# luisrui/Multimodal-Relation-Extrapolation

Hardware: AMD Instinct MI355X
Metric: scored triples/sec + hit@10 parity, FB15K-237-ZS TransE d=200 at 1/2/4/8 MI355X (higher is better)
Workload: dtype f32; 1 GPU; C2 FB15K-237-ZS TransE d=200 p=1 norm_flag, filtered link prediction; n_entities=14208, dim=200, n_sweeps=35192

## Files before the change

multimodal-relation-extrapolation_amd/csrc/link.hip:

```cpp
#include <stdlib.h>

#include <algorithm>
#include <map>
#include <mutex>
#include <tuple>
#include <type_traits>

#include "mmre_common.h"

namespace mmre {

typedef float f32x2 __attribute__((ext_vector_type(2)));

constexpr int TQ = 128;
constexpr int TE = 128;
constexpr int KC = 8;
constexpr int NT = 256;

constexpr int KS_MFMA = 16;
__host__ __device__ inline int n_planes(int model) { return (model == MMRE_COMPLEX || model == MMRE_ROTATE) ? 2 : 1; }
__host__ __device__ inline bool mfma_model(int model) { return model == MMRE_DISTMULT || model == MMRE_COMPLEX; }
inline int plane_rows(int model, int dim) {
  return (int)round_up(dim, !mfma_model(model) ? KC : KS_MFMA / n_planes(model));
}
// ... 655 lines not shown
                                                     const int64_t* __restrict__ off, const int32_t* __restrict__ ids,
                                                     const float* __restrict__ list_v,
                                                     const int32_t* __restrict__ qtrue, const float* __restrict__ thr,
                                                     const int64_t* __restrict__ qr, const int8_t* __restrict__ qmode,
                                                     int64_t n_query, int64_t n_ent,
                                                     const uint32_t* __restrict__ type_head,
                                                     const uint32_t* __restrict__ type_tail, int64_t type_words,
                                                     int32_t* __restrict__ counts) {
  __shared__ __attribute__((aligned(16))) int32_t s_id[64];
  __shared__ __attribute__((aligned(16))) float s_v[64];
  __shared__ __attribute__((aligned(16))) int32_t s_tb[64];
  const int tid = threadIdx.x;
  for (int64_t g = blockIdx.x; g < n_groups; g += gridDim.x) {
    const int64_t qa = grp_qoff[g], qb = grp_qoff[g + 1];
    const int64_t la = off[g], lb = off[g + 1];
    const int64_t q0 = grp_q[qa];
    const uint32_t* tm = type_head ? (qmode[q0] == MMRE_HEAD_BATCH ? type_head : type_tail) : nullptr;
    const int64_t r = qr[q0];
    for (int64_t qc = qa; qc < qb; qc += 64) {
      const int64_t qi = qc + tid;
      const bool active = qi < qb;
      const int64_t q = active ? grp_q[qi] : 0;
      const int32_t tr = active ? qtrue[q] : -1;
      const float th = active ? thr[q] : 0.0f;
      int c = 0, cc = 0;
      for (int64_t lc = la; lc < lb; lc += 64) {
        const int nl = (int)((lb - lc) < 64 ? (lb - lc) : 64);
        __syncthreads();
        {
          int32_t id = -1, tb = 0;
          float v = 0.0f;
          if (tid < nl) {
            const int64_t j = ids[lc + tid];
            if (j >= 0 && j < n_ent) {
              id = (int32_t)j;
              v = list_v[lc + tid];
              tb = tm ? (int32_t)type_bit(tm, type_words, r, j) : 0;
            }
          }
          s_id[tid] = id;
          s_v[tid] = v;
          s_tb[tid] = tb;
        }
        __syncthreads();
        if (active) {
          for (int i = 0; i < nl; i += 4) {
            const int4 e = *reinterpret_cast<const int4*>(&s_id[i]);
            const float4 v = *reinterpret_cast<const float4*>(&s_v[i]);
            const int4 t = *reinterpret_cast<const int4*>(&s_tb[i]);
            const int b0 = (e.x >= 0) & (e.x != tr) & (v.x < th);
            const int b1 = (e.y >= 0) & (e.y != tr) & (v.y < th);
            const int b2 = (e.z >= 0) & (e.z != tr) & (v.z < th);
            const int b3 = (e.w >= 0) & (e.w != tr) & (v.w < th);
            c += b0 + b1 + b2 + b3;
            cc += (b0 & t.x) + (b1 & t.y) + (b2 & t.z) + (b3 & t.w);
          }
        }
      }
      if (active) {
        counts[0 * n_query + q] = 0;
        counts[1 * n_query + q] = -c;
        counts[2 * n_query + q] = 0;
        counts[3 * n_query + q] = -cc;
      }
    }
  }
}

struct UnitMap {
  int m, r, ex0, el0, n_main, lo0, count, nq;
  bool emajor;
  __device__ __forceinline__ UnitMap(int grp, int n_groups, int n_qt, int n_et, bool emajor_ = false) {
    nq = n_qt;
    emajor = emajor_;
    m = n_et / n_groups;
    r = n_et - m * n_groups;
    ex0 = grp * m;
    el0 = m * n_groups;
    n_main = n_qt * m;
    const int64_t left = (int64_t)n_qt * r;
    lo0 = (int)(left * grp / n_groups);
    count = n_main + (int)(left * (grp + 1) / n_groups) - lo0;
  }
  __device__ __forceinline__ void at(int i, int& qt, int& et) const {
    if (i < n_main) {
      if (emajor) {
        qt = i % nq;
        et = ex0 + i / nq;
      } else {
        qt = i / m;
        et = ex0 + i % m;
      }
    } else {
      const int j = lo0 + (i - n_main);
      qt = j / r;
      et = el0 + j % r;
    }
  }
};

struct BlockMap {
  int count, qin, ein, QB, EB, e_lo, n_e;
  __device__ __forceinline__ BlockMap(int grp, int n_groups, int member, int P, int n_qt, int n_et, int qb, int eb) {
    e_lo = (int)((int64_t)n_et * grp / n_groups);
    const int e_hi = (int)((int64_t)n_et * (grp + 1) / n_groups);
    const int m_e = e_hi - e_lo;
    QB = qb;
    EB = eb;
    qin = member / EB;
    ein = member - qin * EB;
    count = 0;
    n_e = 0;
    if (qin >= QB || m_e <= 0) return;
    n_e = ein < m_e ? (m_e - ein + EB - 1) / EB : 0;
    const int n_q = qin < n_qt ? (n_qt - qin + QB - 1) / QB : 0;
    count = n_q * n_e;
  }
  __device__ __forceinline__ void at(int i, int& qt, int& et) const {
    const int a = i / n_e, b = i - a * n_e;
    qt = a * QB + qin;
    et = e_lo + b * EB + ein;
  }
};

template <int GS>
struct ValuSmemGrp {
  uint32_t g_ts[GS][TQ];
  uint32_t g_tw[GS][TQ];
  int32_t g_mq[GS][TQ];
  uint32_t g_acc[GS][TQ];
};
template <>
struct ValuSmemGrp<0> {};
constexpr int L1Q_GS = 8;
constexpr double L1Q_GROUP_FRAC = 0.6;

template <int NPL, bool TC, bool LIST, int GS = 0>
struct ValuSmem : ValuSmemGrp<GS> {
  float4 sq[2][NPL][KC][TQ / 4];
  float4 se[2][NPL][KC][TE / 4];
  float s_thr[2][GS ? 1 : TQ];
  int32_t s_true[2][GS ? 1 : TQ];
  int32_t s_rel[2][TC ? TQ : 1];
  int8_t s_mode[2][TC ? TQ : 1];
  std::conditional_t<TC, uint16_t, int32_t> s_cnt[TC ? 2 : 1][GS ? 1 : 8][GS ? 1 : NT];
  uint32_t s_unc[NT / 64];
  uint32_t s_ts[2][GS ? 1 : TQ];
  uint32_t s_tw[2][GS ? 1 : TQ];
  int s_unit;
  uint32_t s_tb[TC ? 2 : 1][TC ? TQ : 1][4];
  int2 s_pairs[LIST ? NT / 64 : 1][LIST ? 128 : 1];
};

template <int OP, bool TC, bool STORE, int PK, int NPL, int DYNC, int GS = 0, bool IDX = false>
__device__ __forceinline__ void sweep_valu_body(
    ValuSmem<NPL, TC, (OP == 5 || OP == 6), GS>& sm, const float* __restrict__ ent_km, int64_t e_pad, int64_t n_ent,
    const float* __restrict__ q_km, int64_t q_pad, int64_t n_query, int kp, int n_et, int e_base, int n_groups,
    int pred_kind, float margin, const float* __restrict__ thr, const int32_t* __restrict__ qtrue,
    const int64_t* __restrict__ qr, const int8_t* __restrict__ qmode, const uint32_t* __restrict__ type_head,
    const uint32_t* __restrict__ type_tail, int64_t type_words, int32_t* __restrict__ counts,
    float* __restrict__ scores, const L1Q& l1) {
  static_assert(NPL == ((OP == 2) ? 2 : 1), "planes");
  constexpr bool L1F = OP == 5 || OP == 6;
  constexpr bool w8 = OP == 6;
  constexpr bool FAST = (OP == 2 || L1F) && !STORE;
  constexpr bool GRP = GS > 0;
  static_assert(!GRP || (L1F && PK == 0 && !TC && !STORE), "the grouped sweep is the plain integer filter's");
  static_assert(!IDX || (OP == 0 && PK == 0 && !TC && !STORE && DYNC == 0 && !GRP),
                "the indexed sweep is the plain f32 one");
  auto& sq = sm.sq;
  auto& se = sm.se;
  auto& s_thr = sm.s_thr;
  auto& s_true = sm.s_true;
  auto& s_rel = sm.s_rel;
  auto& s_mode = sm.s_mode;
  auto& s_cnt = sm.s_cnt;

  const int tid = threadIdx.x;
  const int tq = tid >> 4, te = tid & 15;
  const PredSel<PK> pred(pred_kind, margin);
  const int grp = blockIdx.x % n_groups, gmem = blockIdx.x / n_groups;
  const int per_grp = gridDim.x / n_groups;
  const int n_idx = IDX ? __builtin_amdgcn_readfirstlane((int)*l1.route_n) : 0;
  const int n_qt = IDX   ? (n_idx + TQ - 1) / TQ
                   : GRP ? __builtin_amdgcn_readfirstlane(l1.n_rows[GRP ? 1 : 0]) / TQ
                         : (int)(q_pad / TQ);
  const UnitMap um(grp, n_groups, n_qt, n_et);
  const int nkc = kp / KC;
  constexpr bool dyn = DYNC > 0;
  constexpr int ch_log2 = DYNC >= 4 ? 2 : DYNC >= 2 ? 1 : 0;
  constexpr int ch_mask = (1 << ch_log2) - 1;
  const int u0 = dyn ? gmem << ch_log2 : (int)((int64_t)gmem * um.count / per_grp);
  const int u1 = dyn ? um.count : (int)((int64_t)(gmem + 1) * um.count / per_grp);
  if (u0 >= u1) return;

  float l1d = 0.0f, l1f = 0.0f, l1c = 0.0f;
  if constexpr (L1F) {
    l1d = __uint_as_float(__builtin_amdgcn_readfirstlane(__float_as_uint(l1q_delta(l1.hdr, w8 ? 255.0f : 65535.0f))));
    l1f = (float)(l1.kt + 4) * 0x1p-23f * (1.0f + 0x1p-8f);
    l1c = __builtin_fmaf((float)l1.kt * 1.03f, l1d, 0x1p-120f);
  }

  auto load_meta = [&](int qtile, int slot) {
    const int tid = vgpr_opaque(threadIdx.x);
    if (tid < TQ) {
      int64_t q = (int64_t)qtile * TQ + tid;
      bool v = q < n_query;
      if constexpr (IDX) {
        v = q < (int64_t)n_idx;
        q = v ? l1.route_list[q] : 0;
      }
      const float th = v ? thr[q] : -INFINITY;
      s_thr[slot][tid] = th;
      s_true[slot][tid] = v ? qtrue[q] : -1;
      if constexpr (L1F && PK == 0) {
        uint32_t t_sure, t_span;
        const bool tight = w8 && l1.q_l1c != nullptr;
        const int ktm = sgpr_opaque(l1.kt);
        const float md = __uint_as_float(sgpr_opaque(__float_as_uint(l1d)));
        const float mf = (float)(ktm + 4) * 0x1p-23f * (1.0f + 0x1p-8f);
        const float mc = __builtin_fmaf((float)ktm * 1.03f, md, 0x1p-120f);
        l1_int_thresholds(th, tight ? (v ? l1.q_l1c[q] : 0.0f) + 0x1p-120f : mc, md, mf, tight ? 2u * l1.hdr[3] : 0u,
                          t_sure, t_span);
        if constexpr (w8) {
          if (l1.routed != nullptr && v && l1.routed[q]) t_sure = t_span = 0u;
        }
        sm.s_ts[slot][tid] = t_sure;
        sm.s_tw[slot][tid] = t_span;
      }
      if constexpr (TC) {
        s_rel[slot][tid] = v ? (int32_t)qr[q] : 0;
        s_mode[slot][tid] = v ? qmode[q] : 0;
      }
    }
  };

  auto load_meta_grp = [&](int qtile) -> int {
    int m = 0;
    if constexpr (GRP) {
      const int tid = vgpr_opaque(threadIdx.x);
      m = min(__builtin_amdgcn_readfirstlane(l1.tile_m[qtile]), GS);
      const bool tight = w8 && l1.q_l1c != nullptr;
      const int ktm = sgpr_opaque(l1.kt);
      const float md = __uint_as_float(sgpr_opaque(__float_as_uint(l1d)));
      const float mf = (float)(ktm + 4) * 0x1p-23f * (1.0f + 0x1p-8f);
      const float mc = __builtin_fmaf((float)ktm * 1.03f, md, 0x1p-120f);
      const uint32_t om2 = tight ? 2u * l1.hdr[3] : 0u;
      static_assert(NT == 2 * TQ && GS % 2 == 0, "two slots' rows per pass");
      const int r = tid % TQ, s0 = tid / TQ;
      const int64_t row = (int64_t)qtile * TQ + r;
      const int cnt = l1.row_cnt[row];
      const int64_t off = l1.row_off[row];
      const float rc = tight ? l1.q_l1c[row] : 0.0f;
      int q[GS / 2];
      float th[GS / 2];
#pragma unroll
      for (int u = 0; u < GS / 2; ++u) {
        q[u] = -1;
        if (s0 + 2 * u < cnt) {
          const int qq = l1.grp_q[off + s0 + 2 * u];
          q[u] = (uint32_t)qq < (uint32_t)n_query ? qq : -1;
        }
      }
      if constexpr (w8) {
        if (l1.routed != nullptr) {
#pragma unroll
          for (int u = 0; u < GS / 2; ++u)
            if (q[u] >= 0 && l1.routed[q[u]]) q[u] = -1;
        }
      }
#pragma unroll
      for (int u = 0; u < GS / 2; ++u) th[u] = q[u] >= 0 ? thr[q[u]] : -INFINITY;
#pragma unroll
      for (int u = 0; u < GS / 2; ++u) {
        const int sl = s0 + 2 * u;
        if (sl < m) {
          uint32_t t_sure, t_span;
          l1_int_thresholds(th[u], tight ? (q[u] >= 0 ? rc : 0.0f) + 0x1p-120f : mc, md, mf, om2, t_sure, t_span);
          sm.g_ts[GRP ? sl : 0][r] = t_sure;
          sm.g_tw[GRP ? sl : 0][r] = t_span;
          sm.g_mq[GRP ? sl : 0][r] = q[u];
        }
      }
    }
    return m;
  };

  const int srow = tid >> 5, sc4 = tid & 31;
  float4 rq0, re0, rq1, re1;
  int ld_unit = u0, ld_kc = 0, ld_qt, ld_et;
  um.at(u0, ld_qt, ld_et);
  uint32_t rt0 = 0u, rt1 = 0u;
  bool st_new = false;
  int ld_tpar = 1, st_par = 0, ep_par = 0;
  [[maybe_unused]] int iq0 = 0, iq1 = 0, iq2 = 0, iq3 = 0;
  auto gload = [&]() {
    if constexpr (TC) {
      st_new = ld_kc == 0;
      if (st_new) {
        ld_tpar ^= 1;
        st_par = ld_tpar;
        const int tt = vgpr_opaque(threadIdx.x);
        const int rr = tt >> 1, jw = tt & 1;
        const int64_t q = (int64_t)ld_qt * TQ + rr;
        uint32_t w0 = 0u, w1 = 0u;
        if (q < n_query) {
          const uint32_t* tm = (qmode[q] == MMRE_HEAD_BATCH ? type_head : type_tail) + qr[q] * type_words;
          const int64_t wb = (e_base + (int64_t)ld_et * TE) >> 5;
          if (wb + jw < type_words) w0 = tm[wb + jw];
          if (wb + 2 + jw < type_words) w1 = tm[wb + 2 + jw];
        }
        rt0 = w0;
        rt1 = w1;
      }
    }
    const int k = ld_kc * KC + srow;
    const int64_t q0 = (int64_t)ld_qt * TQ, e0 = (int64_t)ld_et * TE;
    const float* qp = q_km + (int64_t)k * q_pad + q0 + sc4 * 4;
    const float* ep = ent_km + (int64_t)k * e_pad + e0 + sc4 * 4;
    if constexpr (IDX) {
      if (ld_kc == 0) {
        const int p0 = (int)q0 + sc4 * 4;
        iq0 = p0 + 0 < n_idx ? l1.route_list[p0 + 0] : 0;
        iq1 = p0 + 1 < n_idx ? l1.route_list[p0 + 1] : 0;
        iq2 = p0 + 2 < n_idx ? l1.route_list[p0 + 2] : 0;
        iq3 = p0 + 3 < n_idx ? l1.route_list[p0 + 3] : 0;
      }
      const float* qk = q_km + (int64_t)k * q_pad;
      rq0 = make_float4(qk[iq0], qk[iq1], qk[iq2], qk[iq3]);
    } else {
      rq0 = *reinterpret_cast<const float4*>(qp);
    }
    re0 = *reinterpret_cast<const float4*>(ep);
    if constexpr (NPL == 2) {
      rq1 = *reinterpret_cast<const float4*>(qp + (int64_t)kp * q_pad);
      re1 = *reinterpret_cast<const float4*>(ep + (int64_t)kp * e_pad);
    }
    if (++ld_kc == nkc) {
      ld_kc = 0;
      if (dyn) {
        ld_unit = ((ld_unit + 1) & ch_mask) != 0 ? ld_unit + 1 : sm.s_unit;
        if (ld_unit < u1) um.at(ld_unit, ld_qt, ld_et);
      } else if (++ld_unit < u1) {
        um.at(ld_unit, ld_qt, ld_et);
      }
    }
  };
  auto swrite = [&](int buf) {
    if constexpr (TC) {
      if (st_new) {
        const int tt = vgpr_opaque(threadIdx.x);
        *reinterpret_cast<uint2*>(&sm.s_tb[st_par][tt >> 1][(tt & 1) * 2]) = make_uint2(rt0, rt1);
      }
    }
    sq[buf][0][srow][sc4] = rq0;
    se[buf][0][srow][sc4] = re0;
    if constexpr (NPL == 2) {
      sq[buf][NPL - 1][srow][sc4] = rq1;
      se[buf][NPL - 1][srow][sc4] = re1;
    }
  };

  float acc[8][8];
#pragma unroll
  for (int i = 0; i < 8; ++i)
#pragma unroll
    for (int j = 0; j < 8; ++j) acc[i][j] = 0.0f;
  f32x2 accp[4][8];
#pragma unroll
  for (int i = 0; i < 4; ++i)
#pragma unroll
    for (int j = 0; j < 8; ++j) accp[i][j] = f32x2{0.0f, 0.0f};
  if constexpr (GRP) {
    for (int idx = tid; idx < GS * TQ; idx += NT) (&sm.g_acc[0][0])[idx] = 0u;
  } else {
#pragma unroll
    for (int i = 0; i < 8; ++i) {
      s_cnt[0][i][tid] = 0;
      if constexpr (TC) s_cnt[TC ? 1 : 0][i][tid] = 0;
    }
  }
  if (L1F && tid < NT / 64) sm.s_unc[tid] = 0u;
  constexpr bool LIST = L1F;
  int list_n = 0;
  uint32_t n_listed = 0;
  auto rescore = [&](int2 p, bool active) {
    const int64_t q = p.x;
    const int e = p.y;
    bool ok = active;
    if (active && ((uint64_t)q >= (uint64_t)n_query || (uint32_t)e >= (uint32_t)n_ent)) {
      if (l1.guard) atomicAdd(l1.guard, 1u);
      ok = false;
    }
    if constexpr (GRP) {
      if (ok && e + e_base == qtrue[q]) ok = false;
      n_listed += (uint32_t)__builtin_popcountll(__ballot(ok));
    }
    bool beat = false;
    if (ok) {
      if (l1.und_q) atomicAdd(&l1.und_q[q], 1u);
      const float th = thr[q];
      const float sx = l1_exact_rows<GRP ? 3 : 5>(l1.q_rows + q * (int64_t)l1.kt,
                                                  l1.ent_rows + (int64_t)(e + e_base) * l1.kt, l1.kt);
      beat = pred(sx) < th;
      if constexpr (TC) {
        const uint32_t* tm = qmode[q] == MMRE_HEAD_BATCH ? type_head : type_tail;
        if (beat && type_bit(tm, type_words, qr[q], e + e_base)) atomicAdd(&counts[2 * n_query + q], 1);
      }
    }
    const int qi = (int)q;
    uint64_t pend = __ballot(beat);
    while (pend) {
      const int leader = __builtin_ctzll(pend);
      const int ql = __builtin_amdgcn_readlane(qi, leader);
      const bool mine = beat && qi == ql;
      const uint64_t same = __ballot(mine);
      if ((int)(threadIdx.x & 63) == leader) atomicAdd(&counts[ql], (int)__builtin_popcountll(same));
      if (mine) beat = false;
      pend &= ~same;
    }
  };

  int cur_qt, cur_et;
  um.at(u0, cur_qt, cur_et);
  int slot = 0;
  uint32_t lo = 0xFFFFFFFFu;
  const int kk_last = L1F ? ((((l1.kt + (w8 ? 3 : 1)) >> (w8 ? 2 : 1)) + (w8 ? 2 : 1)) & ~1) - (nkc - 1) * KC
                          : KC;
  const uint32_t fb_flag = L1F ? l1.hdr[1] : 0u;
  int cur_m = 0;
  if constexpr (GRP) cur_m = load_meta_grp(cur_qt);
  else load_meta(cur_qt, 0);
  gload();
  swrite(0);
  __syncthreads();
  if (L1F && __builtin_amdgcn_readfirstlane(fb_flag) != (w8 ? L1Q_CODES8 : L1Q_CODES16)) return;
  if (dyn && ch_mask == 0) {
    if (tid == 0) sm.s_unit = per_grp + (int)atomicAdd(&l1.wq[grp * L1Q_WQ_STRIDE], 1u);
    __syncthreads();
  }

  constexpr int KKU = 2;
  int buf = 0;
  for (int unit = u0; unit < u1;) {
    int unit_next = unit + 1;
    for (int kc = 0; kc < nkc; ++kc) {
      const bool more = ld_unit < u1;
      if (more) gload();
      const int kk_n = (L1F && kc == nkc - 1) ? kk_last : KC;
#pragma unroll KKU
      for (int kk = 0; kk < kk_n; ++kk) {
        float4 a0 = sq[buf][0][kk][tq], a1 = sq[buf][0][kk][16 + tq];
        float4 x0 = se[buf][0][kk][te], x1 = se[buf][0][kk][16 + te];
        const float qa[8] = {a0.x, a0.y, a0.z, a0.w, a1.x, a1.y, a1.z, a1.w};
        const float xv[8] = {x0.x, x0.y, x0.z, x0.w, x1.x, x1.y, x1.z, x1.w};
        if constexpr (OP == 2 && FAST) {
          float4 b0 = sq[buf][NPL - 1][kk][tq], b1 = sq[buf][NPL - 1][kk][16 + tq];
          float4 y0 = se[buf][NPL - 1][kk][te], y1 = se[buf][NPL - 1][kk][16 + te];
          const f32x2 qa2[4] = {{a0.x, a0.y}, {a0.z, a0.w}, {a1.x, a1.y}, {a1.z, a1.w}};
          const f32x2 qb2[4] = {{b0.x, b0.y}, {b0.z, b0.w}, {b1.x, b1.y}, {b1.z, b1.w}};
          const f32x2 xv2[4] = {{x0.x, x0.y}, {x0.z, x0.w}, {x1.x, x1.y}, {x1.z, x1.w}};
          const f32x2 yv2[4] = {{y0.x, y0.y}, {y0.z, y0.w}, {y1.x, y1.y}, {y1.z, y1.w}};
#pragma unroll
          for (int ip = 0; ip < 4; ++ip)
#pragma unroll
            for (int jp = 0; jp < 4; ++jp) {
              const f32x2 dr0 = qa2[ip] - xv2[jp], dr1 = qa2[ip] - xv2[jp].yx;
              const f32x2 di0 = qb2[ip] - yv2[jp], di1 = qb2[ip] - yv2[jp].yx;
              const f32x2 p0 = dr0 * dr0, p1 = dr1 * dr1;
              const f32x2 v0 = __builtin_elementwise_fma(di0, di0, p0), v1 = __builtin_elementwise_fma(di1, di1, p1);
              const f32x2 m0 = {__builtin_amdgcn_sqrtf(v0.x), __builtin_amdgcn_sqrtf(v0.y)};
              const f32x2 m1 = {__builtin_amdgcn_sqrtf(v1.x), __builtin_amdgcn_sqrtf(v1.y)};
              accp[ip][2 * jp] = accp[ip][2 * jp] + m0;
              accp[ip][2 * jp + 1] = accp[ip][2 * jp + 1] + m1;
            }
        } else if constexpr (OP == 2) {
          float4 b0 = sq[buf][NPL - 1][kk][tq], b1 = sq[buf][NPL - 1][kk][16 + tq];
          float4 y0 = se[buf][NPL - 1][kk][te], y1 = se[buf][NPL - 1][kk][16 + te];
          const float qb[8] = {b0.x, b0.y, b0.z, b0.w, b1.x, b1.y, b1.z, b1.w};
          const float yv[8] = {y0.x, y0.y, y0.z, y0.w, y1.x, y1.y, y1.z, y1.w};
          float v[8], y[8];
#pragma unroll
          for (int j = 0; j < 8; ++j) {
            const float dr = qa[0] - xv[j], di = qb[0] - yv[j];
            v[j] = __builtin_fmaf(di, di, dr * dr);
// ... 208 lines not shown
            }
            s_cnt[0][i][tid] += c;
            if constexpr (TC) s_cnt[TC ? 1 : 0][i][tid] += cc;
          }
          if constexpr (LIST) {
            int2* wl = sm.s_pairs[tid >> 6];
            const int lane = tid & 63;
            for (;;) {
              const bool has = (unc[0] | unc[1]) != 0u;
              if (__ballot(has) == 0) break;
              bool keep = false;
              int2 pr = make_int2(0, 0);
              if (has) {
                const int h = unc[0] ? 0 : 1;
                const int p = __builtin_clz(unc[h]);
                unc[h] &= ~(0x80000000u >> p);
                const int i = h * 4 + (p >> 3), j = p & 7;
                const int ql = (i < 4) ? tq * 4 + i : 64 + tq * 4 + (i - 4);
                const int e = (int)ebase + ((j < 4) ? te * 4 + j : 64 + te * 4 + (j - 4));
                keep = (int)(e + e_base) != s_true[slot][ql];
                pr = make_int2((int)(q0 + ql), e);
              }
              const uint64_t bal = __ballot(keep);
              if (keep) {
                const int pos = list_n + (int)__builtin_amdgcn_mbcnt_hi((uint32_t)(bal >> 32),
                                                                       __builtin_amdgcn_mbcnt_lo((uint32_t)bal, 0u));
                wl[pos] = pr;
              }
              const int nb = __builtin_popcountll(bal);
              list_n += nb;
              n_listed += (uint32_t)nb;
              if (list_n >= 64) {
                list_n -= 64;
                rescore(wl[list_n + lane], true);
              }
            }
          }
#pragma unroll
          for (int h = 0; h < 2; ++h) {
            uint32_t m = LIST ? 0u : unc[h];
            while (m) {
              const int p = __builtin_clz(m);
              m &= ~(0x80000000u >> p);
              const int i = h * 4 + (p >> 3), j = p & 7;
              const int ql = (i < 4) ? tq * 4 + i : 64 + tq * 4 + (i - 4);
              const int e = (int)ebase + ((j < 4) ? te * 4 + j : 64 + te * 4 + (j - 4));
              float sx;
              if constexpr (L1F) {
                ++n_listed;
                sx = l1_exact_rows(l1.q_rows + (q0 + ql) * (int64_t)l1.kt, l1.ent_rows + (int64_t)(e + e_base) * l1.kt,
                                   l1.kt);
              } else {
                sx = rot_exact(q_km, q_pad, q0 + ql, ent_km, e_pad, e, kp);
              }
              const float v = pred(sx);
              if (v < s_thr[slot][ql]) {
                s_cnt[0][i][tid] += 1;
                if constexpr (TC) {
                  const uint32_t* tm = s_mode[slot][ql] == MMRE_HEAD_BATCH ? type_head : type_tail;
                  s_cnt[TC ? 1 : 0][i][tid] += type_bit(tm, type_words, s_rel[slot][ql], e + e_base) ? 1 : 0;
                }
              }
            }
          }
#pragma unroll
          for (int i = 0; i < 8; ++i)
#pragma unroll
            for (int j = 0; j < 8; ++j) acc[i][j] = 0.0f;
        } else {
        if constexpr (OP == 2) {
          bool bad = lo < __float_as_uint(kRotMin);
#pragma unroll
          for (int i = 0; i < 8; ++i)
#pragma unroll
            for (int j = 0; j < 8; ++j) bad |= acc[i][j] != acc[i][j];
          if (__ballot(bad)) {
#pragma unroll
            for (int i = 0; i < 8; ++i)
#pragma unroll
              for (int j = 0; j < 8; ++j) acc[i][j] = 0.0f;
            for (int k = 0; k < kp; ++k) {
              float qa[8], qb[8], xv[8], yv[8];
#pragma unroll
              for (int i = 0; i < 8; ++i) {
                const int64_t ql = q0 + ((i < 4) ? tq * 4 + i : 64 + tq * 4 + (i - 4));
                const int64_t ec = ebase + ((i < 4) ? te * 4 + i : 64 + te * 4 + (i - 4));
                qa[i] = q_km[(int64_t)k * q_pad + ql];
                qb[i] = q_km[(int64_t)(kp + k) * q_pad + ql];
                xv[i] = ent_km[(int64_t)k * e_pad + ec];
                yv[i] = ent_km[(int64_t)(kp + k) * e_pad + ec];
              }
#pragma unroll
              for (int i = 0; i < 8; ++i)
#pragma unroll
                for (int j = 0; j < 8; ++j) acc[i][j] = op_step<2>(acc[i][j], qa[i], qb[i], xv[j], yv[j]);
            }
          }
          lo = 0xFFFFFFFFu;
        }
#pragma unroll
        for (int i = 0; i < 8; ++i) {
          const int ql = (i < 4) ? tq * 4 + i : 64 + tq * 4 + (i - 4);
          const float th = s_thr[slot][ql];
          const int32_t tr = s_true[slot][ql];
          int c = 0, cc = 0;
          const uint32_t tb = TC ? tbits(ql) : 0u;
#pragma unroll
          for (int j = 0; j < 8; ++j) {
            const int e = (int)ebase + ((j < 4) ? te * 4 + j : 64 + te * 4 + (j - 4));
            const float v = pred(op_final<OP>(acc[i][j]));
            const bool better = (v < th) & (e + e_base != tr) & (e < n_ent);
            c += better;
            if constexpr (TC) cc += better & ((tb >> j) & 1u);
            if constexpr (STORE) {
              if (q0 + ql < n_query && e < n_ent) scores[(q0 + ql) * n_ent + e] = v;
            }
            acc[i][j] = 0.0f;
          }
          s_cnt[0][i][tid] += c;
          if constexpr (TC) s_cnt[TC ? 1 : 0][i][tid] += cc;
        }
        }
        if (dyn) unit_next = ld_unit;
        const bool last = unit_next >= u1;
        int next_qt = cur_qt, next_et = cur_et;
        if (!last) um.at(unit_next, next_qt, next_et);
        if constexpr (GRP) {
          if (last || next_qt != cur_qt) {
            __syncthreads();
            const int tid = vgpr_opaque(threadIdx.x);
            for (int idx = tid; idx < cur_m * TQ; idx += NT) {
              const uint32_t c = (&sm.g_acc[0][0])[idx];
              if (c) {
                const int q = (&sm.g_mq[0][0])[idx];
                if (q >= 0) atomicAdd(&counts[q], (int)c);
                (&sm.g_acc[0][0])[idx] = 0u;
              }
            }
            if (!last) cur_m = load_meta_grp(next_qt);
          }
        } else
        if (last || next_qt != cur_qt || (TC && n_et > 8 * 8190)) {
          const int tid = vgpr_opaque(threadIdx.x);
          const int tq = tid >> 4, te = tid & 15;
#pragma unroll
          for (int i = 0; i < 8; ++i) {
            int c = s_cnt[0][i][tid], cc = TC ? s_cnt[TC ? 1 : 0][i][tid] : 0;
#pragma unroll
            for (int sh = 1; sh < 16; sh <<= 1) {
              c += __shfl_xor(c, sh);
              if constexpr (TC) cc += __shfl_xor(cc, sh);
            }
            const int ql = (i < 4) ? tq * 4 + i : 64 + tq * 4 + (i - 4);
            int64_t q = q0 + ql;
            bool vq = q < n_query;
            if constexpr (IDX) {
              vq = q < (int64_t)n_idx;
              q = (vq && te == 0) ? l1.route_list[q] : 0;
            }
            if (te == 0 && vq) {
              if (c) atomicAdd(&counts[q], c);
              if constexpr (TC) {
                if (cc) atomicAdd(&counts[2 * n_query + q], cc);
              }
            }
            s_cnt[0][i][tid] = 0;
            if constexpr (TC) s_cnt[TC ? 1 : 0][i][tid] = 0;
          }
          if (!last) {
            slot ^= 1;
            load_meta(next_qt, slot);
          }
        }
        if (dyn && !last && ((unit_next + 1) & ch_mask) == 0 && threadIdx.x == 0)
          sm.s_unit = (per_grp + (int)atomicAdd(&l1.wq[grp * L1Q_WQ_STRIDE], 1u)) << ch_log2;
        if constexpr (TC) ep_par ^= 1;
        cur_qt = next_qt;
        cur_et = next_et;
      }
      if (more) swrite(buf ^ 1);
      __syncthreads();
      buf ^= 1;
    }
    unit = unit_next;
  }
  if constexpr (L1F) {
    if constexpr (LIST) {
      if (list_n > 0) rescore(sm.s_pairs[tid >> 6][tid & 63], (tid & 63) < list_n);
      if ((tid & 63) == 0) sm.s_unc[tid >> 6] = n_listed;
    } else {
      if (n_listed) atomicAdd(&sm.s_unc[tid >> 6], n_listed);
    }
    __syncthreads();
    if (tid == 0) {
      uint32_t t = 0;
#pragma unroll
      for (int w = 0; w < NT / 64; ++w) t += sm.s_unc[w];
      if (t) atomicAdd(reinterpret_cast<uint32_t*>(l1.undecided + (blockIdx.x & (L1Q_SLOTS - 1)) * L1Q_SLOT_STRIDE), t);
    }
  }
}

template <int OP, bool TC, bool STORE, int PK, int DYNC = 0, int GS = 0, bool IDX = false>
__global__ __launch_bounds__(NT, (OP == 2) ? 3 : 4) void k_sweep_valu(
    const float* __restrict__ ent_km, int64_t e_pad, int64_t n_ent, const float* __restrict__ q_km,
    int64_t q_pad, int64_t n_query, int kp, int n_et, int e_base, int n_groups, int pred_kind, float margin,
    const float* __restrict__ thr, const int32_t* __restrict__ qtrue, const int64_t* __restrict__ qr,
    const int8_t* __restrict__ qmode, const uint32_t* __restrict__ type_head,
    const uint32_t* __restrict__ type_tail, int64_t type_words, int32_t* __restrict__ counts,
    float* __restrict__ scores, L1Q l1) {
  constexpr int NPL = (OP == 2) ? 2 : 1;
  __shared__ ValuSmem<NPL, TC, (OP == 5 || OP == 6), GS> sm;
  if (l1.gate != nullptr) {
    const uint32_t want = OP == 6 ? L1Q_CODES8 : OP == 5 ? L1Q_CODES16 : L1Q_F32;
    if (__builtin_amdgcn_readfirstlane(*l1.gate) != want) {
      if (l1.fin_counts != nullptr) {
        for (int64_t q = (int64_t)blockIdx.x * NT + threadIdx.x; q < l1.fin_n; q += (int64_t)gridDim.x * NT) {
          l1.fin_counts[l1.fin_n + q] += l1.fin_counts[q];
          if constexpr (TC) l1.fin_counts[3 * l1.fin_n + q] += l1.fin_counts[2 * l1.fin_n + q];
        }
      }
      return;
    }
  }
  sweep_valu_body<OP, TC, STORE, PK, NPL, DYNC, GS, IDX>(sm, ent_km, e_pad, n_ent, q_km, q_pad, n_query, kp, n_et, e_base,
                                          n_groups, pred_kind, margin, thr, qtrue, qr, qmode, type_head, type_tail,
                                          type_words, counts, scores, l1);
  if (l1.gate != nullptr && l1.fin_counts != nullptr) {
    __shared__ uint32_t s_last;
    __asm__ volatile("s_waitcnt vmcnt(0)" ::: "memory");
    __syncthreads();
    if (threadIdx.x == 0)
      s_last = __hip_atomic_fetch_add(l1.fin_ticket, 1u, __ATOMIC_RELAXED, __HIP_MEMORY_SCOPE_AGENT) == gridDim.x - 1;
    __syncthreads();
    if (s_last) {
      for (int64_t q = threadIdx.x; q < l1.fin_n; q += NT) {
        atomicAdd(&l1.fin_counts[l1.fin_n + q],
                  __hip_atomic_load(&l1.fin_counts[q], __ATOMIC_RELAXED, __HIP_MEMORY_SCOPE_AGENT));
        if constexpr (TC)
          atomicAdd(&l1.fin_counts[3 * l1.fin_n + q],
                    __hip_atomic_load(&l1.fin_counts[2 * l1.fin_n + q], __ATOMIC_RELAXED, __HIP_MEMORY_SCOPE_AGENT));
      }
      if (threadIdx.x == 0) *l1.fin_ticket = 0u;
    }
  }
}

__global__ __launch_bounds__(256) void k_counts_finalize(int32_t* __restrict__ counts, int64_t n_query, int tc) {
  const int64_t q = (int64_t)blockIdx.x * blockDim.x + threadIdx.x;
  if (q >= n_query) return;
  counts[n_query + q] += counts[q];
  if (tc) counts[3 * n_query + q] += counts[2 * n_query + q];
}

typedef float floatx16 __attribute__((ext_vector_type(16)));

template <bool TC, bool STORE, int PK, int KS>
__global__ __launch_bounds__(NT, KS == 16 && !TC && !STORE ? 4 : 2) void k_sweep_mfma(
    const float* __restrict__ ent_km, int64_t e_pad, int64_t n_ent, const float* __restrict__ q_km,
    int64_t q_pad, int64_t n_query, int ktot, int n_et, int e_base, int n_groups, int pred_kind, float margin,
    const float* __restrict__ thr, const int64_t* __restrict__ qr, const int8_t* __restrict__ qmode,
    const uint32_t* __restrict__ type_head, const uint32_t* __restrict__ type_tail, int64_t type_words,
    int32_t* __restrict__ counts, float* __restrict__ scores, int emajor, const uint32_t* __restrict__ gate) {
  static_assert(KS == 16 || KS == 32, "stage of 16 or 32 K rows");
  if (gate != nullptr && *gate == 0u) return;
  constexpr bool BAL = KS == 16;
  __shared__ float sq[2][KS][TQ];
  __shared__ float se[2][KS][TE];
  __shared__ int32_t s_rel[TC ? TQ : 1];
  __shared__ int8_t s_mode[TC ? TQ : 1];
  __shared__ __attribute__((aligned(16))) float s_th[2][TQ];

  const int tid = threadIdx.x;
  const int lane = tid & 63, wave = tid >> 6;
  const PredSel<PK> pred(pred_kind, margin);
  const int wq = wave >> 1, we = wave & 1;
  const int lrow = lane >> 5, lcol = lane & 31;
  const int grp = blockIdx.x % n_groups, gmem = blockIdx.x / n_groups;
  const int per_grp = gridDim.x / n_groups;
  const UnitMap um(grp, n_groups, (int)(q_pad / TQ), n_et, emajor != 0);
  const int u0 = (int)((int64_t)gmem * um.count / per_grp);
  const int u1 = (int)((int64_t)(gmem + 1) * um.count / per_grp);
  if (u0 >= u1) return;
  const int nkc = (ktot + KS - 1) / KS;
  const bool half_tail = KS == 32 && (ktot % 32) != 0;

  int tpar = 0;
  int cntv = 0, cntv_tc = 0;
  int cnt[BAL ? 1 : 2][BAL ? 1 : 16], cnt_tc[TC && !BAL ? 2 : 1][TC && !BAL ? 16 : 1];
  auto row_of = [&](int bi, int r) { return wq * 64 + bi * 32 + (r & 3) + 8 * (r >> 2) + 4 * lrow; };
  auto load_rows = [&](int qtile) {
    const int64_t q0 = (int64_t)qtile * TQ;
    tpar ^= 1;
    if (tid < TQ) {
      const int64_t q = q0 + tid;
      s_th[tpar][tid] = q < n_query ? thr[q] : -INFINITY;
    }
    cntv = 0;
    cntv_tc = 0;
    if constexpr (!BAL) {
#pragma unroll
      for (int bi = 0; bi < 2; ++bi)
#pragma unroll
        for (int r = 0; r < 16; ++r) {
          cnt[bi][r] = 0;
          if constexpr (TC) cnt_tc[bi][r] = 0;
        }
    }
    if constexpr (TC) {
      __syncthreads();
      if (tid < TQ) {
        const int64_t q = q0 + tid;
        s_rel[tid] = q < n_query ? (int32_t)qr[q] : 0;
        s_mode[tid] = q < n_query ? qmode[q] : 0;
      }
    }
  };
  auto flush_rows = [&](int qtile) {
    if constexpr (BAL) {
      const int64_t q = (int64_t)qtile * TQ + wq * 64 + lane;
      if (q < n_query) {
        if (cntv) atomicAdd(&counts[q], cntv);
        if constexpr (TC) {
          if (cntv_tc) atomicAdd(&counts[2 * n_query + q], cntv_tc);
        }
      }
    } else {
      const int64_t q0 = (int64_t)qtile * TQ;
#pragma unroll
      for (int bi = 0; bi < 2; ++bi)
#pragma unroll
        for (int r = 0; r < 16; ++r) {
          int c = cnt[bi][r];
#pragma unroll
          for (int sh = 1; sh < 32; sh <<= 1) c += __shfl_xor(c, sh);
          int cc = 0;
          if constexpr (TC) {
            cc = cnt_tc[bi][r];
#pragma unroll
            for (int sh = 1; sh < 32; sh <<= 1) cc += __shfl_xor(cc, sh);
          }
          const int64_t q = q0 + row_of(bi, r);
          if (lcol == 0 && q < n_query) {
            if (c) atomicAdd(&counts[q], c);
            if constexpr (TC) {
              if (cc) atomicAdd(&counts[2 * n_query + q], cc);
            }
          }
        }
    }
  };

  const int srow = tid >> 5, sc4 = tid & 31;
  float4 rq0, rq1, re0, re1, rq2, rq3, re2, re3;
  int ld_unit = u0, ld_kc = 0, ld_qt, ld_et;
  um.at(u0, ld_qt, ld_et);
  auto gload = [&]() {
    const int k = ld_kc * KS + srow;
    const float* qp = q_km + (int64_t)k * q_pad + (int64_t)ld_qt * TQ + sc4 * 4;
    const float* ep = ent_km + (int64_t)k * e_pad + (int64_t)ld_et * TE + sc4 * 4;
    rq0 = *reinterpret_cast<const float4*>(qp);
    rq1 = *reinterpret_cast<const float4*>(qp + 8 * q_pad);
    re0 = *reinterpret_cast<const float4*>(ep);
    re1 = *reinterpret_cast<const float4*>(ep + 8 * e_pad);
    if (KS == 32 && !(half_tail && ld_kc == nkc - 1)) {
      rq2 = *reinterpret_cast<const float4*>(qp + 16 * q_pad);
      rq3 = *reinterpret_cast<const float4*>(qp + 24 * q_pad);
      re2 = *reinterpret_cast<const float4*>(ep + 16 * e_pad);
      re3 = *reinterpret_cast<const float4*>(ep + 24 * e_pad);
    }
    if (++ld_kc == nkc) {
      ld_kc = 0;
      if (++ld_unit < u1) um.at(ld_unit, ld_qt, ld_et);
    }
  };
  auto swrite = [&](int buf) {
    *reinterpret_cast<float4*>(&sq[buf][srow][sc4 * 4]) = rq0;
    *reinterpret_cast<float4*>(&sq[buf][srow + 8][sc4 * 4]) = rq1;
    *reinterpret_cast<float4*>(&se[buf][srow][sc4 * 4]) = re0;
    *reinterpret_cast<float4*>(&se[buf][srow + 8][sc4 * 4]) = re1;
    if constexpr (KS == 32) {
      *reinterpret_cast<float4*>(&sq[buf][srow + 16][sc4 * 4]) = rq2;
      *reinterpret_cast<float4*>(&sq[buf][srow + 24][sc4 * 4]) = rq3;
      *reinterpret_cast<float4*>(&se[buf][srow + 16][sc4 * 4]) = re2;
      *reinterpret_cast<float4*>(&se[buf][srow + 24][sc4 * 4]) = re3;
    }
  };

  floatx16 acc[2][2];
#pragma unroll
  for (int a = 0; a < 2; ++a)
#pragma unroll
    for (int b = 0; b < 2; ++b)
#pragma unroll
      for (int r = 0; r < 16; ++r) acc[a][b][r] = 0.0f;

  int cur_qt, cur_et;
  um.at(u0, cur_qt, cur_et);
  load_rows(cur_qt);
  gload();
  swrite(0);
  __syncthreads();

  int buf = 0;
  for (int unit = u0; unit < u1; ++unit) {
// ... 2588 lines not shown
                                      int64_t e_pad, float* d_ent_rows, float* d_q_km, int64_t q_pad, float* d_q_rows,
                                      int32_t* d_q_true, float* d_list_scores, int32_t* d_counts, float* d_truth,
                                      uint32_t* d_undecided_q, void* d_work, int64_t work_bytes, void* stream) {
  if (!d_ent || !d_rel || !d_qh || !d_qr || !d_qt || !d_qmode || !d_ent_km || !d_ent_rows || !d_q_km || !d_q_rows ||
      !d_q_true || !d_counts || !d_truth || !d_grp_qoff || !d_grp_q || !d_filt_off)
    return MMRE_ERR_ARG;
  if (n_ent <= 0 || n_rel <= 0 || dim <= 0 || n_query <= 0 || n_groups <= 0 || n_groups > n_query || n_entries < 0)
    return MMRE_ERR_ARG;
  if (e_pad < n_ent || e_pad % TE || q_pad < n_query || q_pad % TQ) return MMRE_ERR_ARG;
  const int kp = plane_rows(MMRE_TRANSE_L1, dim), kt = kp;
  SweepCall C{(hipStream_t)stream, d_ent_km, e_pad, d_q_km, q_pad, n_query, 0, 0.0f, d_truth, d_q_true, d_qr, d_qmode};
  C.counts = d_counts;
  if (int rc = sweep_slice(C, n_ent, e_begin, e_end, kp); rc) return rc;
  if (n_entries > 0 && (!d_filt_ids || !d_entry_q || !d_list_scores)) return MMRE_ERR_WORKSPACE;
  if (n_ent > (int64_t)INT32_MAX - 256 || n_query >= (int64_t)INT32_MAX) return MMRE_ERR_SHAPE;
  EvalWork W;
  if (!d_work || work_bytes < eval_layout(W, dim, e_pad, q_pad, d_work)) return MMRE_ERR_WORKSPACE;
  hipStream_t st = C.st;
  const int rb = eval_rb(kp), rbq = eval_rbq(kp);
  const size_t lds1 = sizeof(float) * (size_t)std::max(rb, 3 * rbq) * (kt + 1);
  if (lds1 > 64 * 1024) return MMRE_ERR_SHAPE;
  const L1QWork& WQ = W.q;
  const char* cap_env = getenv("MMRE_GROUP_CAP");
  int row_cap = cap_env ? std::min(L1Q_GS, std::max(1, atoi(cap_env))) : L1Q_GS;
  if (!cap_env) {
    const int64_t res = resident_groups((const void*)k_sweep_valu<6, false, false, 0, 1, L1Q_GS>, NT);
    const int64_t rows8 = std::min<int64_t>(n_query, n_groups + n_query / L1Q_GS);
    if ((rows8 + TQ - 1) / TQ * C.n_et < res || (double)rows8 > L1Q_GROUP_FRAC * (double)n_query) row_cap = 0;
  }
  const bool grouped = row_cap > 0;
  const int64_t rows_max = grouped ? std::min<int64_t>(n_query, n_groups + n_query / row_cap) : n_query;
  static const char* tight_env = getenv("MMRE_L1_TIGHT");
  const int bits = l1q_bits();
  const bool tight = kt <= 1984 && !(tight_env && tight_env[0] == '0');
  EvalL1 P{};
  P.ent = d_ent;
  P.rel = d_rel;
  P.n_ent = n_ent;
  P.dim = dim;
  P.kp = kp;
  P.norm = norm_flag ? 1 : 0;
  P.rb = rb;
  P.rbq = rbq;
  P.qh = d_qh;
  P.qr = d_qr;
  P.qt = d_qt;
  P.qmode = d_qmode;
  P.n_query = n_query;
  P.ent_km = d_ent_km;
  P.e_pad = e_pad;
  P.ent_rows = d_ent_rows;
  P.q_km = d_q_km;
  P.q_pad = q_pad;
  P.q_rows = d_q_rows;
  P.q_true = d_q_true;
  P.truth = d_truth;
  P.e_begin = e_begin;
  P.e_cols = C.e_cols;
  P.n_eblk = (int)((e_pad + rb - 1) / rb);
  P.n_qblk = (int)((q_pad + rbq - 1) / rbq);
  P.pstat = W.pstat;
  P.und_q = d_undecided_q;
  P.ticket = W.ticket;
  P.hdr = WQ.hdr;
  P.n_elem = (double)kp * (double)(q_pad + C.e_cols);
  P.ratio = l1q_ratio();
  P.grp_qoff = d_grp_qoff;
  P.n_groups = n_groups;
  P.row_cap = row_cap;
  P.row_off = W.row_off;
  P.row_cnt = W.row_cnt;
  P.tile_m = W.tile_m;
  P.n_rows = W.n_rows;
  hipLaunchKernelGGL(k_eval_prep, dim3((unsigned)((grouped ? 1 : 0) + P.n_eblk + P.n_qblk)), dim3(256), lds1, st, P);
  MMRE_CHECK_LAUNCH();
  EvalQuant Q{};
  Q.pq = L1QPlane{d_q_km, q_pad, 0, q_pad, WQ.vq};
  Q.pe = L1QPlane{d_ent_km, e_pad, e_begin, C.e_cols, WQ.ve};
  Q.out16q = WQ.uq;
  Q.out16e = WQ.ue;
  Q.kw = WQ.k4;
  Q.k2 = WQ.k2;
  Q.kt = kt;
  const int n_lblk = (int)((n_entries + 255) / 256);
  Q.n_blk = (int)std::min<int64_t>(512, std::max<int64_t>(64, (resident_groups((const void*)k_eval_quant_list, 256) -
                                                              n_lblk) / 2));
  Q.tight = tight ? 1 : 0;
  Q.q_l1c = WQ.q_l1c;
  Q.row_off = W.row_off;
  Q.row_cnt = W.row_cnt;
  Q.grp_q = d_grp_q;
  Q.n_rows = grouped ? W.n_rows : nullptr;
  Q.row_of_q = W.row_of_q;
  Q.tile_m = W.tile_m;
  const int n_mblk = grouped ? (int)((rows_max + 255) / 256) : 0;
  hipLaunchKernelGGL(k_eval_quant_list, dim3((unsigned)(n_lblk + 2 * Q.n_blk + n_mblk)), dim3(256), 0, st, P, Q, d_filt_ids,
                     d_entry_q, n_entries, d_list_scores, n_lblk);
  MMRE_CHECK_LAUNCH();
  const RouteStore R = route_store(W.pstat, dim, e_pad, q_pad, n_query);
  const char* heavy_env = getenv("MMRE_L1_HEAVY");
  bool heavy = bits != 16 && R.cap > 0;
  if (heavy && heavy_env) heavy = atoi(heavy_env) != 0;
  else if (heavy) {
    const int64_t res = resident_groups((const void*)k_sweep_valu<6, false, false, 0, 1, L1Q_GS>, NT);
    const int64_t rows8 = std::min<int64_t>(n_query, n_groups + n_query / L1Q_GS);
    heavy = bits == 0 && (rows8 + TQ - 1) / TQ * C.n_et >= res;
  }
  HeavyProbe H{};
  uint32_t route_cap = 0;
  if (heavy) {
    const char* min_env = getenv("MMRE_L1_HEAVY_MIN");
    const char* cap_env2 = getenv("MMRE_L1_HEAVY_CAP");
    const uint32_t n_samp = l1q_heavy_sample(C.n_slice);
    H.n_blk = (int)((rows_max + 31) / 32);
    H.e_base = C.e_base;
    H.row_off = grouped ? W.row_off : nullptr;
    H.row_cnt = grouped ? W.row_cnt : nullptr;
    H.n_rows = grouped ? W.n_rows : nullptr;
    H.flags = R.flags;
    H.min_count = min_env ? (uint32_t)std::min<long long>(std::max(0LL, atoll(min_env)), UINT32_MAX)
                          : std::max<uint32_t>(1u, (uint32_t)std::ceil(L1Q_HEAVY_FRAC * (double)n_samp));
    route_cap = (uint32_t)(cap_env2 ? std::min<long long>(std::max(0LL, atoll(cap_env2)), R.cap_store) : R.cap);
  }
  const int n_cblk = (int)std::min<int64_t>((n_groups + 3) / 4, 65536);
  const uint32_t probe_max = l1q_probe_max(C.n_slice);
  hipLaunchKernelGGL(k_eval_count_probe, dim3((unsigned)(n_cblk + L1Q_PROBE_Q / 4 + H.n_blk)), dim3(256), 0, st,
                     d_grp_qoff, d_grp_q, n_groups, n_cblk, d_filt_off, d_filt_ids, d_list_scores, d_q_true, d_truth,
                     n_query, n_ent, d_counts, WQ.vq, q_pad, WQ.ve + e_begin, e_pad, C.n_slice, WQ.k4, kt,
                     tight ? WQ.q_l1c : nullptr, WQ.hdr, W.ticket, probe_max, bits == 8 || bits == 16 ? bits : 0,
                     grouped ? W.row_of_q : nullptr, H);
  MMRE_CHECK_LAUNCH();
  if (heavy) {
    const double cost = std::ceil(L1Q_HEAVY_ROW_COST * (double)C.n_slice / L1Q_PAIR_COST);
    hipLaunchKernelGGL(k_l1q_route_compact, dim3(1), dim3(1024), 0, st, WQ.hdr, R.flags, R.list, n_query, q_pad,
                       route_cap, d_undecided_q, (uint32_t)cost, l1q_heavy_sample(C.n_slice), H.min_count);
    MMRE_CHECK_LAUNCH();
  }
  L1Q l1 = l1q_operands(WQ, C, d_q_rows, d_ent_rows, tight, d_undecided_q);
  if (grouped) {
    l1.row_off = W.row_off;
    l1.row_cnt = W.row_cnt;
    l1.grp_q = d_grp_q;
    l1.tile_m = W.tile_m;
    l1.n_rows = W.n_rows;
  }
  if (heavy) l1.routed = R.flags;
  L1Q l16 = l1;
  l16.gate = WQ.hdr + 1;
  const SweepCall C8 = planes(C, WQ.ve, WQ.vq, WQ.k4), C16 = planes(C, WQ.ue, WQ.uq, WQ.k2);
  int rc = grouped ? launch_valu_grp<6>(C8, l1, rows_max) : launch_valu<6>(C8, l1, false);
  if (!rc) rc = grouped ? launch_valu_grp<5>(C16, l16, rows_max) : launch_valu<5>(C16, l16, false);
  if (rc) return rc;
  if (heavy && route_cap > 0) {
    L1Q lr{};
    lr.route_list = R.list;
    lr.route_n = WQ.hdr + L1Q_ROUTE_W + 1;
    const void* kh = (const void*)k_sweep_valu<0, false, false, 0, 0, 0, true>;
    const int64_t units = sweep_units(((int64_t)route_cap + TQ - 1) / TQ, C.n_et);
    const int g = (int)std::max<int64_t>(1, std::min<int64_t>(resident_groups(kh, NT), units));
    hipLaunchKernelGGL((k_sweep_valu<0, false, false, 0, 0, 0, true>), dim3((unsigned)g), dim3(NT), 0, st, C.ent, C.e_pad,
                       C.n_slice, C.q, C.q_pad, C.n_query, C.kp, C.n_et, C.e_base, xcd_groups(g, C.n_et), 0, 0.0f,
                       C.truth, C.q_true, nullptr, nullptr, nullptr, nullptr, (int64_t)0, C.counts, nullptr, lr);
    MMRE_CHECK_LAUNCH();
  }
  L1Q gate{};
  gate.gate = WQ.hdr + 1;
  gate.fin_counts = d_counts;
  gate.fin_n = n_query;
  gate.fin_ticket = WQ.hdr + 6;
  return launch_valu<0>(C, gate, false);
}
```

Measured before the change: 788.1 billion scored triples/s.

## Replace indexed VALU sweep for routed heavy queries with dedicated row kernel

Removes the IDX variant of the tiled VALU sweep, which gathered routed query rows through an index list inside a 128-query tile. In its place is a dedicated kernel that handles 16 routed queries per block against a 128-entity tile. Query rows are read row-major with wave-uniform addresses, entity columns are prefetched 8 K-rows ahead, and counts come from ballot/popcount. This is meant to avoid wasting large query tiles when few queries are routed, and to cut the cost of gathered loads. The trade-off is lower reuse of entity data per block when many queries are routed.

```diff
diff --git a/multimodal-relation-extrapolation_amd/csrc/link.hip b/multimodal-relation-extrapolation_amd/csrc/link.hip
--- a/multimodal-relation-extrapolation_amd/csrc/link.hip
+++ b/multimodal-relation-extrapolation_amd/csrc/link.hip
@@ -831,7 +831,7 @@
   int2 s_pairs[LIST ? NT / 64 : 1][LIST ? 128 : 1];
 };
 
-template <int OP, bool TC, bool STORE, int PK, int NPL, int DYNC, int GS = 0, bool IDX = false>
+template <int OP, bool TC, bool STORE, int PK, int NPL, int DYNC, int GS = 0>
 __device__ __forceinline__ void sweep_valu_body(
     ValuSmem<NPL, TC, (OP == 5 || OP == 6), GS>& sm, const float* __restrict__ ent_km, int64_t e_pad, int64_t n_ent,
     const float* __restrict__ q_km, int64_t q_pad, int64_t n_query, int kp, int n_et, int e_base, int n_groups,
@@ -845,8 +845,6 @@
   constexpr bool FAST = (OP == 2 || L1F) && !STORE;
   constexpr bool GRP = GS > 0;
   static_assert(!GRP || (L1F && PK == 0 && !TC && !STORE), "the grouped sweep is the plain integer filter's");
-  static_assert(!IDX || (OP == 0 && PK == 0 && !TC && !STORE && DYNC == 0 && !GRP),
-                "the indexed sweep is the plain f32 one");
   auto& sq = sm.sq;
   auto& se = sm.se;
   auto& s_thr = sm.s_thr;
@@ -860,10 +858,7 @@
   const PredSel<PK> pred(pred_kind, margin);
   const int grp = blockIdx.x % n_groups, gmem = blockIdx.x / n_groups;
   const int per_grp = gridDim.x / n_groups;
-  const int n_idx = IDX ? __builtin_amdgcn_readfirstlane((int)*l1.route_n) : 0;
-  const int n_qt = IDX   ? (n_idx + TQ - 1) / TQ
-                   : GRP ? __builtin_amdgcn_readfirstlane(l1.n_rows[GRP ? 1 : 0]) / TQ
-                         : (int)(q_pad / TQ);
+  const int n_qt = GRP ? __builtin_amdgcn_readfirstlane(l1.n_rows[GRP ? 1 : 0]) / TQ : (int)(q_pad / TQ);
   const UnitMap um(grp, n_groups, n_qt, n_et);
   const int nkc = kp / KC;
   constexpr bool dyn = DYNC > 0;
@@ -883,12 +878,8 @@
   auto load_meta = [&](int qtile, int slot) {
     const int tid = vgpr_opaque(threadIdx.x);
     if (tid < TQ) {
-      int64_t q = (int64_t)qtile * TQ + tid;
-      bool v = q < n_query;
-      if constexpr (IDX) {
-        v = q < (int64_t)n_idx;
-        q = v ? l1.route_list[q] : 0;
-      }
+      const int64_t q = (int64_t)qtile * TQ + tid;
+      const bool v = q < n_query;
       const float th = v ? thr[q] : -INFINITY;
       s_thr[slot][tid] = th;
       s_true[slot][tid] = v ? qtrue[q] : -1;
@@ -972,7 +963,6 @@
   uint32_t rt0 = 0u, rt1 = 0u;
   bool st_new = false;
   int ld_tpar = 1, st_par = 0, ep_par = 0;
-  [[maybe_unused]] int iq0 = 0, iq1 = 0, iq2 = 0, iq3 = 0;
   auto gload = [&]() {
     if constexpr (TC) {
       st_new = ld_kc == 0;
@@ -997,19 +987,7 @@
     const int64_t q0 = (int64_t)ld_qt * TQ, e0 = (int64_t)ld_et * TE;
     const float* qp = q_km + (int64_t)k * q_pad + q0 + sc4 * 4;
     const float* ep = ent_km + (int64_t)k * e_pad + e0 + sc4 * 4;
-    if constexpr (IDX) {
-      if (ld_kc == 0) {
-        const int p0 = (int)q0 + sc4 * 4;
-        iq0 = p0 + 0 < n_idx ? l1.route_list[p0 + 0] : 0;
-        iq1 = p0 + 1 < n_idx ? l1.route_list[p0 + 1] : 0;
-        iq2 = p0 + 2 < n_idx ? l1.route_list[p0 + 2] : 0;
-        iq3 = p0 + 3 < n_idx ? l1.route_list[p0 + 3] : 0;
-      }
-      const float* qk = q_km + (int64_t)k * q_pad;
-      rq0 = make_float4(qk[iq0], qk[iq1], qk[iq2], qk[iq3]);
-    } else {
-      rq0 = *reinterpret_cast<const float4*>(qp);
-    }
+    rq0 = *reinterpret_cast<const float4*>(qp);
     re0 = *reinterpret_cast<const float4*>(ep);
     if constexpr (NPL == 2) {
       rq1 = *reinterpret_cast<const float4*>(qp + (int64_t)kp * q_pad);
@@ -1524,12 +1502,8 @@
               if constexpr (TC) cc += __shfl_xor(cc, sh);
             }
             const int ql = (i < 4) ? tq * 4 + i : 64 + tq * 4 + (i - 4);
-            int64_t q = q0 + ql;
-            bool vq = q < n_query;
-            if constexpr (IDX) {
-              vq = q < (int64_t)n_idx;
-              q = (vq && te == 0) ? l1.route_list[q] : 0;
-            }
+            const int64_t q = q0 + ql;
+            const bool vq = q < n_query;
             if (te == 0 && vq) {
               if (c) atomicAdd(&counts[q], c);
               if constexpr (TC) {
@@ -1573,7 +1547,7 @@
   }
 }
 
-template <int OP, bool TC, bool STORE, int PK, int DYNC = 0, int GS = 0, bool IDX = false>
+template <int OP, bool TC, bool STORE, int PK, int DYNC = 0, int GS = 0>
 __global__ __launch_bounds__(NT, (OP == 2) ? 3 : 4) void k_sweep_valu(
     const float* __restrict__ ent_km, int64_t e_pad, int64_t n_ent, const float* __restrict__ q_km,
     int64_t q_pad, int64_t n_query, int kp, int n_et, int e_base, int n_groups, int pred_kind, float margin,
@@ -1595,9 +1569,9 @@
       return;
     }
   }
-  sweep_valu_body<OP, TC, STORE, PK, NPL, DYNC, GS, IDX>(sm, ent_km, e_pad, n_ent, q_km, q_pad, n_query, kp, n_et, e_base,
-                                          n_groups, pred_kind, margin, thr, qtrue, qr, qmode, type_head, type_tail,
-                                          type_words, counts, scores, l1);
+  sweep_valu_body<OP, TC, STORE, PK, NPL, DYNC, GS>(sm, ent_km, e_pad, n_ent, q_km, q_pad, n_query, kp, n_et, e_base,
+                                                    n_groups, pred_kind, margin, thr, qtrue, qr, qmode, type_head, type_tail,
+                                                    type_words, counts, scores, l1);
   if (l1.gate != nullptr && l1.fin_counts != nullptr) {
     __shared__ uint32_t s_last;
     __asm__ volatile("s_waitcnt vmcnt(0)" ::: "memory");
@@ -1623,6 +1597,69 @@
   if (q >= n_query) return;
   counts[n_query + q] += counts[q];
   if (tc) counts[3 * n_query + q] += counts[2 * n_query + q];
+}
+
+constexpr int HR_TE = 128;
+constexpr int HR_QB = 16;
+constexpr int HR_KU = 8;
+static_assert(HR_TE == TE && HR_KU == KC && HR_TE % 64 == 0 && HR_QB <= HR_TE, "routed rows' unit");
+__global__ __launch_bounds__(HR_TE) void k_heavy_rows(
+    const float* __restrict__ ent_km, int64_t e_pad, int64_t n_ent, int n_et, int e_base,
+    const float* __restrict__ q_rows, int kp, const float* __restrict__ thr, const int32_t* __restrict__ qtrue,
+    const int32_t* __restrict__ route_list, const uint32_t* __restrict__ route_n, int32_t* __restrict__ counts) {
+  __shared__ int s_cnt[HR_TE / 64][HR_QB];
+  const int tid = threadIdx.x;
+  const int n_idx = __builtin_amdgcn_readfirstlane((int)*route_n);
+  const int n_qb = (n_idx + HR_QB - 1) / HR_QB;
+  const int64_t units = (int64_t)n_qb * n_et;
+  for (int64_t unit = blockIdx.x; unit < units; unit += gridDim.x) {
+    const int et = (int)(unit / n_qb), p0 = (int)(unit % n_qb) * HR_QB;
+    const float* qp[HR_QB];
+    float th[HR_QB];
+    int32_t tr[HR_QB];
+#pragma unroll
+    for (int i = 0; i < HR_QB; ++i) {
+      const bool v = p0 + i < n_idx;
+      const int q = __builtin_amdgcn_readfirstlane(route_list[v ? p0 + i : p0]);
+      qp[i] = q_rows + (int64_t)q * kp;
+      th[i] = v ? thr[q] : -INFINITY;
+      tr[i] = qtrue[q];
+    }
+    const int e = et * HR_TE + tid;
+    const float* ep = ent_km + e;
+    float acc[HR_QB];
+#pragma unroll
+    for (int i = 0; i < HR_QB; ++i) acc[i] = 0.0f;
+    float ev[HR_KU], en[HR_KU];
+#pragma unroll
+    for (int u = 0; u < HR_KU; ++u) ev[u] = en[u] = ep[(int64_t)u * e_pad];
+    for (int k0 = 0; k0 < kp; k0 += HR_KU) {
+      if (k0 + HR_KU < kp) {
+#pragma unroll
+        for (int u = 0; u < HR_KU; ++u) en[u] = ep[(int64_t)(k0 + HR_KU + u) * e_pad];
+      }
+#pragma unroll
+      for (int u = 0; u < HR_KU; ++u)
+#pragma unroll
+        for (int i = 0; i < HR_QB; ++i) acc[i] = op_step<0>(acc[i], qp[i][k0 + u], 0.0f, ev[u], 0.0f);
+#pragma unroll
+      for (int u = 0; u < HR_KU; ++u) ev[u] = en[u];
+    }
+#pragma unroll
+    for (int i = 0; i < HR_QB; ++i) {
+      const bool better = (op_final<0>(acc[i]) < th[i]) & (e + e_base != tr[i]) & (e < n_ent);
+      const int c = __popcll(__ballot(better));
+      if ((tid & 63) == 0) s_cnt[tid >> 6][i] = c;
+    }
+    __syncthreads();
+    if (tid < HR_QB && p0 + tid < n_idx) {
+      int c = 0;
+#pragma unroll
+      for (int w = 0; w < HR_TE / 64; ++w) c += s_cnt[w][tid];
+      if (c) atomicAdd(&counts[route_list[p0 + tid]], c);
+    }
+    __syncthreads();
+  }
 }
 
 typedef float floatx16 __attribute__((ext_vector_type(16)));
@@ -4517,15 +4554,12 @@
   if (!rc) rc = grouped ? launch_valu_grp<5>(C16, l16, rows_max) : launch_valu<5>(C16, l16, false);
   if (rc) return rc;
   if (heavy && route_cap > 0) {
-    L1Q lr{};
-    lr.route_list = R.list;
-    lr.route_n = WQ.hdr + L1Q_ROUTE_W + 1;
-    const void* kh = (const void*)k_sweep_valu<0, false, false, 0, 0, 0, true>;
-    const int64_t units = sweep_units(((int64_t)route_cap + TQ - 1) / TQ, C.n_et);
-    const int g = (int)std::max<int64_t>(1, std::min<int64_t>(resident_groups(kh, NT), units));
-    hipLaunchKernelGGL((k_sweep_valu<0, false, false, 0, 0, 0, true>), dim3((unsigned)g), dim3(NT), 0, st, C.ent, C.e_pad,
-                       C.n_slice, C.q, C.q_pad, C.n_query, C.kp, C.n_et, C.e_base, xcd_groups(g, C.n_et), 0, 0.0f,
-                       C.truth, C.q_true, nullptr, nullptr, nullptr, nullptr, (int64_t)0, C.counts, nullptr, lr);
+    const int64_t units = (((int64_t)route_cap + HR_QB - 1) / HR_QB) * C.n_et;
+    const int g = (int)std::max<int64_t>(
+        1, std::min<int64_t>(2 * (int64_t)resident_groups((const void*)k_heavy_rows, HR_TE), units));
+    hipLaunchKernelGGL(k_heavy_rows, dim3((unsigned)g), dim3(HR_TE), 0, st, C.ent, C.e_pad, C.n_slice, C.n_et, C.e_base,
+                       d_q_rows, C.kp, C.truth, C.q_true, (const int32_t*)R.list,
+                       (const uint32_t*)(WQ.hdr + L1Q_ROUTE_W + 1), C.counts);
     MMRE_CHECK_LAUNCH();
   }
   L1Q gate{};
```

Result: faster. 836.6 billion scored triples/s (median of 6 runs) (+6.2%).
